# facebookresearch/esm

Measured on AMD Instinct MI355X. Metric: residues/sec (whole node) ESM-2 650M L=1022 bulk extract, higher is better.
Workload: dtype f16; 1 GPU; esm2_t33_650M_UR50D forward (repr_layers=[33] + logits), synthetic tokens [B,1024], random-init weights of the 650M architecture; batch_per_gpu=64, seq_len=1022, ln_fold=on (library default)

## Files before the change

### esm_amd/csrc/gemm9.hip

```cpp
#include "gemm_epi.h"
#include <type_traits>

namespace esmk {

constexpr int Q_BUF = 65536;
constexpr int Q_WOFF = 32768;
constexpr int Q_EPI = 2 * Q_BUF;
constexpr int Q_SLICE = 8192;
constexpr int Q_LDS = Q_EPI + 4 * Q_SLICE;

#define ESMK_INL __attribute__((always_inline))

template <typename T, int EPI, bool FULL, int D = 4, bool NT = true, int NMI = 8, bool SB = false, bool LNF = false>
ESMK_DEV void epilogue9_f32(const GemmArgs& p, f32x4 (&acc)[8][NMI], int m_base, int n_base, int lane, char* wl) {
    static_assert(!LNF || EPI == EPI_RESID_F32, "the LayerNorm-fold producer is the residual epilogue");
    constexpr bool lnp = LNF;
    constexpr int NP = 2 * NMI;
    constexpr int NIB = NMI / 2;
    float s1[4], s2[4];
    float cmv[2][4];
    typedef unsigned u32x2 __attribute__((ext_vector_type(2)));
    typedef unsigned u32x4 __attribute__((ext_vector_type(4)));
    u32x2 hold[4];
    T* h16 = reinterpret_cast<T*>(p.h16);
    if constexpr (!FULL)
        if (n_base >= p.N || m_base >= p.M) return;
    float* out = reinterpret_cast<float*>(p.out);
    const int ldc = p.N;
    const int g4 = lane >> 4, l16 = lane & 15;
    f32x4 old[D][4];
    constexpr bool SADDR = LNF && FULL;
    int la = lane;
    if constexpr (LNF) asm volatile("" : "+v"(la));
    typedef unsigned long long u64;
    u64 ob = 0, hb = 0, pb = 0, mb = 0;
    unsigned ov[4], hv[4];
    unsigned o_rb = 0, h_rb = 0, p_rb = 0;
    if constexpr (SADDR) {
        ob = (u64)out + ((u64)m_base * (u64)ldc + (u64)n_base) * 4;
        hb = (u64)h16 + ((u64)m_base * (u64)p.ldh + (u64)n_base) * sizeof(T);
        pb = (u64)p.ln_part + ((u64)m_base * (u64)p.ln_parts + (u64)(n_base >> 7)) * 8;
        mb = (u64)(p.ln_mean + m_base);
        o_rb = 32u * (unsigned)ldc, h_rb = 8u * (unsigned)sizeof(T) * (unsigned)p.ldh, p_rb = 64u * (unsigned)p.ln_parts;
        const unsigned r8 = la >> 3, c8 = la & 7;
#pragma unroll
        for (int it = 0; it < 4; ++it) {
            ov[it] = (8u * it + r8) * 4u * (unsigned)ldc + 16u * c8;
            hv[it] = (8u * it + r8) * (unsigned)sizeof(T) * (unsigned)p.ldh + (unsigned)sizeof(T) * ((c8 & 1) ? 32u + 4u * (c8 - 1) : 4u * c8);
        }
    }
    auto gaddr = [](u64 base, int imm, unsigned off, auto* as) ESMK_INL {
        asm("" : "+s"(base));
        typedef typename std::remove_pointer<decltype(as)>::type E;
        return (__attribute__((address_space(1))) E*)(base + (u64)imm + (u64)off);
    };
    auto out_at = [&](int i, int jb, int it) ESMK_INL { return gaddr(ob + (u64)(4 * i) * o_rb, 128 * jb, ov[it], (f32x4*)nullptr); };
    auto load_old = [&](f32x4 (&dst)[4], int piece) ESMK_INL {
        const int i = piece >> 2, jb = piece & 3;
        if constexpr (SADDR) {
#pragma unroll
            for (int it = 0; it < 4; ++it) dst[it] = *out_at(i, jb, it);
            return;
        }
#pragma unroll
        for (int it = 0; it < 4; ++it) {
            const int pc = it * 64 + la;
            const int m = FULL ? m_base + 32 * i + (pc >> 3) : min(m_base + 32 * i + (pc >> 3), p.M - 1);
            const int n = FULL ? n_base + 32 * jb + (pc & 7) * 4 : min(n_base + 32 * jb + (pc & 7) * 4, p.N - 4);
            dst[it] = *reinterpret_cast<const f32x4*>(out + (size_t)m * ldc + n);
        }
    };
    if constexpr (EPI == EPI_RESID_F32) {
#pragma unroll
        for (int d = 0; d < D; ++d) load_old(old[d], d);
    }
    auto load_means = [&](int i) ESMK_INL {
#pragma unroll
        for (int it = 0; it < 4; ++it) {
            const int m = m_base + 32 * i + it * 8 + (la >> 3);
            if constexpr (SADDR)
                cmv[i & 1][it] = (kExperiments && (p.lnf_dbg & 4)) ? 0.f : *gaddr(mb, 4 * (32 * i + 8 * it), 4u * (unsigned)(la >> 3), (const float*)nullptr);
            else
                cmv[i & 1][it] = (kExperiments && (p.lnf_dbg & 4)) ? 0.f : p.ln_mean[FULL ? m : min(m, p.M - 1)];
        }
    };
    if constexpr (LNF)
        if (lnp) load_means(0);
#pragma unroll
    for (int piece = 0; piece < NP; ++piece) {
        const int i = piece >> 2, jb = piece & 3;
        char* sl = wl + (SB ? 0 : (piece & 1) * 4096);
        if constexpr (LNF) {
            if (jb == 0 && lnp) {
#pragma unroll
                for (int it = 0; it < 4; ++it) s1[it] = s2[it] = 0.f;
                if (i + 1 < NIB) load_means(i + 1);
            }
        }
#pragma unroll
        for (int q = 0; q < 4; ++q) {
            const int mi2 = q >> 1, nj2 = q & 1;
            const int row = 16 * mi2 + l16;
            f32x4 v = acc[2 * jb + nj2][2 * i + mi2];
            if constexpr (EPI == EPI_GELU_F32) gelu_fast_x4(v);
            *reinterpret_cast<f32x4*>(sl + row * 128 + (((4 * nj2 + g4) ^ (row & 7)) << 4)) = v;
        }
        f32x4 vv[4];
#pragma unroll
        for (int it = 0; it < 4; ++it) {
            const int pc = it * 64 + lane;
            const int r = pc >> 3, cc = pc & 7;
            vv[it] = *reinterpret_cast<const f32x4*>(sl + r * 128 + ((cc ^ (r & 7)) << 4));
        }
#pragma unroll
        for (int it = 0; it < 4; ++it) {
            const int pc = it * 64 + la;
            const int r = pc >> 3, cc = pc & 7;
            f32x4 v = vv[it];
            if constexpr (EPI == EPI_RESID_F32) {
                const f32x4 o = old[piece % D][it];
                v = f32x4{o[0] + v[0], o[1] + v[1], o[2] + v[2], o[3] + v[3]};
            }
            const int m = m_base + 32 * i + r, n = n_base + 32 * jb + cc * 4;
            const bool inside = FULL || (m < p.M && n < p.N);
            if (inside) {
                if constexpr (SADDR) {
                    if constexpr (NT) __builtin_nontemporal_store(v, out_at(i, jb, it));
                    else *out_at(i, jb, it) = v;
                } else {
                    if constexpr (NT) __builtin_nontemporal_store(v, reinterpret_cast<f32x4*>(out + (size_t)m * ldc + n));
                    else *reinterpret_cast<f32x4*>(out + (size_t)m * ldc + n) = v;
                }
            }
            if (LNF && lnp) {
                const float c = cmv[i & 1][it];
                float d0 = v[0] - c, d1 = v[1] - c, d2 = v[2] - c, d3 = v[3] - c;
                if (!inside) d0 = d1 = d2 = d3 = 0.f;
                s1[it] += (d0 + d1) + (d2 + d3);
                s2[it] = __builtin_fmaf(d3, d3, __builtin_fmaf(d2, d2, __builtin_fmaf(d1, d1, __builtin_fmaf(d0, d0, s2[it]))));
                typename Op<T>::v4 pk;
                pk[0] = Op<T>::from(d0), pk[1] = Op<T>::from(d1), pk[2] = Op<T>::from(d2), pk[3] = Op<T>::from(d3);
                const u32x2 cur = __builtin_bit_cast(u32x2, pk);
                if ((jb & 1) == 0) {
                    hold[it] = cur;
                } else {
                    const bool odd = (lane & 1) != 0;
                    const u32x2 prev = hold[it];
                    const u32x2 send = odd ? prev : cur;
                    u32x2 recv;
                    recv.x = (unsigned)__builtin_amdgcn_update_dpp(0, (int)send.x, 0xB1, 0xf, 0xf, true);
                    recv.y = (unsigned)__builtin_amdgcn_update_dpp(0, (int)send.y, 0xB1, 0xf, 0xf, true);
                    const u32x4 o = odd ? u32x4{recv.x, recv.y, cur.x, cur.y} : u32x4{prev.x, prev.y, recv.x, recv.y};
                    const int col = n_base + ((la & 1) ? 32 * jb + 4 * (cc - 1) : 32 * (jb - 1) + 4 * cc);
                    if ((FULL || (m < p.M && col < p.N)) && !(kExperiments && (p.lnf_dbg & 1))) {
                        if constexpr (SADDR) {
                            auto* hd = gaddr(hb + (u64)(4 * i) * h_rb, 32 * (jb - 1) * (int)sizeof(T), hv[it], (u32x4*)nullptr);
                            if constexpr (NT) __builtin_nontemporal_store(o, hd);
                            else *hd = o;
                        } else {
                            auto* hd = reinterpret_cast<u32x4*>(h16 + (size_t)m * p.ldh + col);
                            if constexpr (NT) __builtin_nontemporal_store(o, hd);
                            else *hd = o;
                        }
                    }
                }
            }
        }
        if constexpr (EPI == EPI_RESID_F32)
            if (piece + D < NP) load_old(old[piece % D], piece + D);
        if constexpr (LNF) {
            if (jb == 3 && lnp && !(kExperiments && (p.lnf_dbg & 2))) {
#pragma unroll
                for (int it = 0; it < 4; ++it) {
                    float a = s1[it], b = s2[it];
                    a += __builtin_bit_cast(float, __builtin_amdgcn_update_dpp(0, __builtin_bit_cast(int, a), 0x111, 0xf, 0xf, true));
                    b += __builtin_bit_cast(float, __builtin_amdgcn_update_dpp(0, __builtin_bit_cast(int, b), 0x111, 0xf, 0xf, true));
                    a += __builtin_bit_cast(float, __builtin_amdgcn_update_dpp(0, __builtin_bit_cast(int, a), 0x112, 0xf, 0xf, true));
                    b += __builtin_bit_cast(float, __builtin_amdgcn_update_dpp(0, __builtin_bit_cast(int, b), 0x112, 0xf, 0xf, true));
                    a += __builtin_bit_cast(float, __builtin_amdgcn_update_dpp(0, __builtin_bit_cast(int, a), 0x114, 0xf, 0xf, true));
                    b += __builtin_bit_cast(float, __builtin_amdgcn_update_dpp(0, __builtin_bit_cast(int, b), 0x114, 0xf, 0xf, true));
                    const int m = m_base + 32 * i + it * 8 + (la >> 3);
                    if ((lane & 7) == 7 && (FULL || m < p.M)) {
                        f32x2 st = {a, b};
                        if constexpr (SADDR) {
                            *gaddr(pb + (u64)(4 * i + it) * p_rb, 0, (unsigned)(la >> 3) * 8u * (unsigned)p.ln_parts, (f32x2*)nullptr) = st;
                        } else {
                            *reinterpret_cast<f32x2*>(p.ln_part + ((size_t)m * p.ln_parts + (n_base >> 7)) * 2) = st;
                        }
                    }
                }
            }
        }
    }
}

template <typename T, int EPI, bool FULL, bool NT = false, int NMI = 8, int RR = 32, bool LNF = false, bool X3O = false>
ESMK_DEV void epilogue9_t(const GemmArgs& p, f32x4 (&acc)[8][NMI], int m_base, int n_base, int lane, char* wl) {
    static_assert(!X3O || (EPI == EPI_GELU_T && !LNF), "hi | hi | lo output rows: the plain GELU epilogue");
    using V8 = typename Op<T>::v8;
    float bs1[8];
    constexpr int LPR = EPI == EPI_QKV_ROPE ? 4 : 8;
    constexpr int RPI = 64 / LPR;
    constexpr int NIT = RR / RPI;
    constexpr int NI_ = NMI * 16 / RR;
    float rsv[LNF ? NI_ : 1][NIT];
    if constexpr (LNF) {
        if (FULL || m_base < p.M) {
#pragma unroll
            for (int i = 0; i < NI_; ++i)
#pragma unroll
                for (int it = 0; it < NIT; ++it) {
                    const int m = m_base + RR * i + RPI * it + lane / LPR;
                    rsv[i][it] = p.ln_rstd[FULL ? m : min(m, p.M - 1)];
                }
        }
    }
    constexpr int NI = NMI * 16 / RR;
    constexpr int NR = 2 * NI;
    constexpr int MB = RR / 16;
    const int g4 = lane >> 4, l16 = lane & 15;
    if constexpr (!FULL)
        if (m_base >= p.M) return;
    constexpr bool ROPE = EPI == EPI_QKV_ROPE;
    constexpr int NV = ROPE ? NI * NIT : 1;
    int rtt[NV];
    unsigned rro[NV];
    f32x4 tab[ROPE ? NIT : 1][4];
    float bsq1[ROPE && LNF ? 2 : 1][8], bsq2[ROPE && LNF ? 2 : 1][8];
    float sch[2] = {1.0f, 1.0f};
    T* qkh[2] = {nullptr, nullptr};
    int headh[2] = {0, 0};
    auto load_tab = [&](int it, int i) ESMK_INL {
        const size_t o = (size_t)rtt[i * NIT + it] * 32 + 8 * (lane & 3);
#pragma unroll
        for (int e2 = 0; e2 < 2; ++e2) {
            tab[it][e2] = *reinterpret_cast<const f32x4*>(p.cos + o + 4 * e2);
            tab[it][2 + e2] = *reinterpret_cast<const f32x4*>(p.sin + o + 4 * e2);
        }
    };
    if constexpr (ROPE) {
#pragma unroll
        for (int v = 0; v < NV; ++v) {
            const int mm = m_base + RR * (v / NIT) + 16 * (v % NIT) + (lane >> 2);
            const int m = FULL ? mm : min(mm, p.M - 1);
            const int b = m / p.T;
            rtt[v] = m - b * p.T;
            rro[v] = (unsigned)(b * p.H) * (unsigned)p.T + (unsigned)rtt[v];
        }
        if (p.row_pos != nullptr) {
#pragma unroll
            for (int v = 0; v < NV; ++v) {
                const int mm = m_base + RR * (v / NIT) + 16 * (v % NIT) + (lane >> 2);
                rtt[v] = p.row_pos[FULL ? mm : min(mm, p.M - 1)];
            }
        }
#pragma unroll
        for (int hf = 0; hf < 2; ++hf) {
            const int nb = n_base + 64 * hf;
            const bool live = FULL || nb < p.N;
            const int which = nb / p.E;
            headh[hf] = (nb - which * p.E) >> 6;
            qkh[hf] = reinterpret_cast<T*>(which == 0 ? p.q : p.k);
            sch[hf] = which == 0 ? p.scaling : 1.0f;
            if constexpr (LNF) {
                const int c0 = (live ? nb : n_base) + 8 * (lane & 3);
                f32x4 a[2], b[2];
#pragma unroll
                for (int e2 = 0; e2 < 2; ++e2)
                    a[e2] = *reinterpret_cast<const f32x4*>(p.bias + c0 + 4 * e2), b[e2] = *reinterpret_cast<const f32x4*>(p.bias + c0 + 32 + 4 * e2);
                if (p.bias2 != nullptr) {
#pragma unroll
                    for (int e2 = 0; e2 < 2; ++e2) {
                        const f32x4 a2 = *reinterpret_cast<const f32x4*>(p.bias2 + c0 + 4 * e2), b2 = *reinterpret_cast<const f32x4*>(p.bias2 + c0 + 32 + 4 * e2);
#pragma unroll
                        for (int e = 0; e < 4; ++e) a[e2][e] += a2[e], b[e2][e] += b2[e];
                    }
                }
#pragma unroll
                for (int e2 = 0; e2 < 2; ++e2)
#pragma unroll
                    for (int e = 0; e < 4; ++e) bsq1[hf][4 * e2 + e] = a[e2][e] * sch[hf], bsq2[hf][4 * e2 + e] = b[e2][e] * sch[hf];
            }
        }
#pragma unroll
        for (int it = 0; it < NIT; ++it) load_tab(it, 0);
    }
    auto write_round = [&](int r) ESMK_INL {
        const int hf = ROPE ? r % 2 : r / NI, i = ROPE ? r / 2 : r % NI;
#pragma unroll
        for (int mi2 = 0; mi2 < MB; ++mi2)
#pragma unroll
            for (int nq = 0; nq < 4; ++nq) {
                const int row = 16 * mi2 + l16, chunk = 4 * nq + g4;
                *reinterpret_cast<f32x4*>(wl + row * 256 + ((chunk ^ (row & 7)) << 4)) = acc[4 * hf + nq][MB * i + mi2];
            }
    };
    auto read_round = [&](f32x4 (&raw)[8]) ESMK_INL {
        if constexpr (EPI == EPI_QKV_ROPE) {
#pragma unroll
            for (int it = 0; it < RR / 16; ++it) {
                const int slot = it * 64 + lane;
                const int r = slot >> 2, g4 = slot & 3;
#pragma unroll
                for (int e2 = 0; e2 < 2; ++e2) {
                    raw[4 * it + e2] = *reinterpret_cast<const f32x4*>(wl + r * 256 + (((2 * g4 + e2) ^ (r & 7)) << 4));
                    raw[4 * it + 2 + e2] = *reinterpret_cast<const f32x4*>(wl + r * 256 + (((8 + 2 * g4 + e2) ^ (r & 7)) << 4));
                }
            }
        } else {
#pragma unroll
            for (int it = 0; it < RR / 8; ++it) {
                const int slot = it * 64 + lane;
                const int r = slot >> 3, c8 = slot & 7;
#pragma unroll
                for (int e2 = 0; e2 < 2; ++e2)
                    raw[2 * it + e2] = *reinterpret_cast<const f32x4*>(wl + r * 256 + (((2 * c8 + e2) ^ (r & 7)) << 4));
            }
        }
    };
    auto finish_round = [&](int rd, const f32x4 (&raw)[8]) ESMK_INL {
        const int hf = ROPE ? rd % 2 : rd / NI, i = ROPE ? rd / 2 : rd % NI;
        const int nb = n_base + 64 * hf;
        if constexpr (ROPE) {
            const bool live = FULL || nb < p.N;
            const float sc = sch[hf];
#pragma unroll
            for (int it = 0; it < NIT; ++it) {
                const int g4 = lane & 3;
                const int mm = m_base + RR * i + 16 * it + (lane >> 2);
                float rs = sc;
                if constexpr (LNF) rs = rsv[i][it] * sc;
                V8 o1, o2;
                if (live) {
                    float y1[8], y2[8];
#pragma unroll
                    for (int e2 = 0; e2 < 2; ++e2) {
                        const f32x4 c = tab[it][e2], s = tab[it][2 + e2];
#pragma unroll
                        for (int e = 0; e < 4; ++e) {
                            const float x1 = LNF ? __builtin_fmaf(raw[4 * it + e2][e], rs, bsq1[LNF ? hf : 0][4 * e2 + e]) : raw[4 * it + e2][e] * sc;
                            const float x2 = LNF ? __builtin_fmaf(raw[4 * it + 2 + e2][e], rs, bsq2[LNF ? hf : 0][4 * e2 + e]) : raw[4 * it + 2 + e2][e] * sc;
                            y1[4 * e2 + e] = __builtin_fmaf(x1, c[e], -(x2 * s[e]));
                            y2[4 * e2 + e] = __builtin_fmaf(x2, c[e], x1 * s[e]);
                        }
                    }
#pragma unroll
                    for (int e = 0; e < 8; ++e) o1[e] = Op<T>::from(y1[e]), o2[e] = Op<T>::from(y2[e]);
                }
                __builtin_amdgcn_sched_barrier(0);
                if (hf == 1 && i + 1 < NI) load_tab(it, i + 1);
                __builtin_amdgcn_sched_barrier(0);
                if (live && (FULL || mm < p.M)) {
                    T* dst = qkh[hf] + ((size_t)rro[i * NIT + it] + (size_t)headh[hf] * p.T) * 64 + 8 * g4;
                    if constexpr (NT) {
                        __builtin_nontemporal_store(o1, reinterpret_cast<V8*>(dst));
                        __builtin_nontemporal_store(o2, reinterpret_cast<V8*>(dst + 32));
                    } else {
                        *reinterpret_cast<V8*>(dst) = o1;
                        *reinterpret_cast<V8*>(dst + 32) = o2;
                    }
                }
            }
        } else {
            if constexpr (!FULL)
                if (nb >= p.N) return;
            T* out = reinterpret_cast<T*>(p.out);
            if constexpr (LNF) {
                if (i == 0) {
                    const int c0 = FULL ? nb + 8 * (lane & 7) : min(nb + 8 * (lane & 7), p.N - 8);
#pragma unroll
                    for (int e2 = 0; e2 < 2; ++e2) {
                        f32x4 a = *reinterpret_cast<const f32x4*>(p.bias + c0 + 4 * e2);
                        if (p.bias2 != nullptr) {
                            const f32x4 a2 = *reinterpret_cast<const f32x4*>(p.bias2 + c0 + 4 * e2);
#pragma unroll
                            for (int e = 0; e < 4; ++e) a[e] += a2[e];
                        }
#pragma unroll
                        for (int e = 0; e < 4; ++e) bs1[4 * e2 + e] = a[e];
                    }
                }
            }
#pragma unroll
            for (int it = 0; it < RR / 8; ++it) {
                const int slot = it * 64 + lane;
                const int r = slot >> 3, c8 = slot & 7;
                float v[8];
#pragma unroll
                for (int e2 = 0; e2 < 2; ++e2)
#pragma unroll
                    for (int e = 0; e < 4; ++e) v[4 * e2 + e] = raw[2 * it + e2][e];
                if constexpr (LNF) {
                    const float rs = rsv[i][it];
#pragma unroll
                    for (int e = 0; e < 8; ++e) v[e] = __builtin_fmaf(v[e], rs, bs1[e]);
                }
                if constexpr (EPI == EPI_GELU_T) gelu_fast_x8<!X3O>(v);
                V8 o;
#pragma unroll
                for (int e = 0; e < 8; ++e) o[e] = Op<T>::from(v[e]);
                const int m = m_base + RR * i + r, n = nb + 8 * c8;
                if constexpr (X3O) {
                    if (FULL || (m < p.M && n < p.N)) {
                        V8 lo;
#pragma unroll
                        for (int e = 0; e < 8; ++e) lo[e] = Op<T>::from(v[e] - Op<T>::to(o[e]));
                        T* q = out + (size_t)m * (3 * (size_t)p.N) + (size_t)(n >> 6) * 192 + (n & 63);
                        *reinterpret_cast<V8*>(q) = o;
                        *reinterpret_cast<V8*>(q + 64) = o;
                        *reinterpret_cast<V8*>(q + 128) = lo;
                    }
                } else
                if (FULL || (m < p.M && n < p.N)) {
                    if constexpr (NT) __builtin_nontemporal_store(o, reinterpret_cast<V8*>(out + (size_t)m * p.N + n));
                    else *reinterpret_cast<V8*>(out + (size_t)m * p.N + n) = o;
                }
            }
        }
    };
    write_round(0);
#pragma unroll
    for (int rd = 0; rd < NR; ++rd) {
        f32x4 raw[8];
        read_round(raw);
        if (rd + 1 < NR) write_round(rd + 1);
        __builtin_amdgcn_sched_barrier(0);
        finish_round(rd, raw);
    }
}

template <typename T, bool FULL, bool NT, int NMI, bool LNF, bool COL0>
ESMK_DEV void epilogue9_vt(const GemmArgs& p, f32x4 (&acc)[8][NMI], int m_base, int n_base, int lane, char* wl, int col0) {
    using V8 = typename Op<T>::v8;
    constexpr int NTH = NMI / 4;
    constexpr int CH = NMI == 8 ? 32 : 16;
    constexpr int NCG = 128 / CH;
    constexpr int NR = NTH * NCG;
    constexpr int NIT = CH / 8;
    const int g4 = lane >> 4, l16 = lane & 15;
    const int c8 = lane & 7, r8 = lane >> 3;
    const int ncols = COL0 ? p.N - col0 : p.N;
    if constexpr (!FULL)
        if (m_base >= p.M || n_base >= ncols) return;
    T* vt = reinterpret_cast<T*>(p.vt);
    const bool aligned = FULL || (p.T % 32 == 0);
    float bvc[NCG][NIT];
#pragma unroll
    for (int cg = 0; cg < NCG; ++cg)
#pragma unroll
        for (int it = 0; it < NIT; ++it) {
            const int n = n_base + CH * cg + 8 * it + r8;
            bvc[cg][it] = p.bias[(COL0 ? col0 : 0) + (FULL ? n : min(n, ncols - 1))];
        }
    if constexpr (LNF) {
        if (p.bias2 != nullptr) {
#pragma unroll
            for (int cg = 0; cg < NCG; ++cg)
#pragma unroll
                for (int it = 0; it < NIT; ++it) {
                    const int n = n_base + CH * cg + 8 * it + r8;
                    bvc[cg][it] += p.bias2[(COL0 ? col0 : 0) + (FULL ? n : min(n, ncols - 1))];
                }
        }
    }
    f32x4 rs[LNF ? NTH : 1][2];
    if constexpr (LNF) {
#pragma unroll
        for (int th = 0; th < NTH; ++th)
#pragma unroll
            for (int e2 = 0; e2 < 2; ++e2)
                rs[th][e2] = *reinterpret_cast<const f32x4*>(p.ln_rstd + m_base + 64 * th + 16 * (c8 >> 1) + 4 * ((c8 & 1) + 2 * e2));
    }
    size_t run[NTH];
#pragma unroll
    for (int th = 0; th < NTH; ++th) {
        const int m = m_base + 64 * th + 8 * c8;
        const int mc = FULL ? m : min(m, p.M - 1);
        const int b = mc / p.T;
        run[th] = (size_t)(b * p.H * 64) * p.Tp + (mc - b * p.T);
    }
    auto write_round = [&](int r) ESMK_INL {
        const int th = r / NCG, cg = r % NCG;
#pragma unroll
        for (int nj2 = 0; nj2 < CH / 16; ++nj2)
#pragma unroll
            for (int mq = 0; mq < 4; ++mq) {
                const int row = 16 * nj2 + l16, chunk = 4 * mq + g4;
                *reinterpret_cast<f32x4*>(wl + row * 256 + ((chunk ^ (row & 7)) << 4)) = acc[(CH / 16) * cg + nj2][4 * th + mq];
            }
    };
    auto read_round = [&](f32x4 (&raw)[2 * NIT]) ESMK_INL {
#pragma unroll
        for (int it = 0; it < NIT; ++it) {
            const int r = 8 * it + r8;
#pragma unroll
            for (int e2 = 0; e2 < 2; ++e2)
                raw[2 * it + e2] = *reinterpret_cast<const f32x4*>(wl + r * 256 + (((4 * (c8 >> 1) + (c8 & 1) + 2 * e2) ^ (r & 7)) << 4));
        }
    };
    size_t eo[8];
    auto finish_round = [&](int rd, const f32x4 (&raw)[2 * NIT]) ESMK_INL {
        const int th = rd / NCG, cg = rd % NCG;
        if constexpr (!FULL) {
            if (n_base + CH * cg >= ncols) return;
            if (!aligned && cg == 0) {
#pragma unroll
                for (int e2 = 0; e2 < 2; ++e2)
#pragma unroll
                    for (int e = 0; e < 4; ++e) {
                        const int m = m_base + 64 * th + 16 * (c8 >> 1) + 4 * ((c8 & 1) + 2 * e2) + e;
                        const int mc = min(m, p.M - 1);
                        const int b = mc / p.T, t = mc - b * p.T;
                        const int t16 = t & 15;
                        const int tp = (t & ~15) | ((((t16 >> 2) & 1) << 3) | (((t16 >> 3) & 1) << 2) | (t16 & 3));
                        eo[4 * e2 + e] = m < p.M ? (size_t)(b * p.H * 64) * p.Tp + tp : ~(size_t)0;
                    }
            }
        }
#pragma unroll
        for (int it = 0; it < NIT; ++it) {
            const int n = n_base + CH * cg + 8 * it + r8;
            const float bv = bvc[cg][it];
            float x[8];
#pragma unroll
            for (int e2 = 0; e2 < 2; ++e2)
#pragma unroll
                for (int e = 0; e < 4; ++e) {
                    if constexpr (LNF) x[4 * e2 + e] = __builtin_fmaf(raw[2 * it + e2][e], rs[th][e2][e], bv);
                    else x[4 * e2 + e] = raw[2 * it + e2][e] + bv;
                }
            asm volatile("" : "+v"(x[0]), "+v"(x[1]), "+v"(x[2]), "+v"(x[3]), "+v"(x[4]), "+v"(x[5]), "+v"(x[6]), "+v"(x[7]));
            V8 o;
#pragma unroll
            for (int e = 0; e < 8; ++e) o[e] = Op<T>::from(x[e]);
            if (aligned) {
                if (FULL || (m_base + 64 * th + 8 * c8 < p.M && n < ncols)) {
                    T* dst = vt + run[th] + (size_t)n * p.Tp;
                    if constexpr (NT) __builtin_nontemporal_store(o, reinterpret_cast<V8*>(dst));
                    else *reinterpret_cast<V8*>(dst) = o;
                }
            } else if constexpr (!FULL) {
                if (n < ncols) {
#pragma unroll
                    for (int e = 0; e < 8; ++e)
                        if (eo[e] != ~(size_t)0) vt[eo[e] + (size_t)n * p.Tp] = o[e];
                }
            }
        }
    };
    write_round(0);
#pragma unroll
    for (int rd = 0; rd < NR; ++rd) {
        f32x4 raw[2 * NIT];
        read_round(raw);
        if (rd + 1 < NR) write_round(rd + 1);
        __builtin_amdgcn_sched_barrier(0);
        finish_round(rd, raw);
    }
}

template <typename T, int EPI, int VAR = 0, bool HM = false, bool LNF = false, bool X3O = false>
__global__ __launch_bounds__(256, 1) void gemm9_kernel(GemmArgs p, unsigned long long* timing) {
    static_assert(!X3O || (EPI == EPI_GELU_T && !HM && !LNF && VAR == 0), "hi | hi | lo output rows: plain full-height GELU kernel");
    static_assert(!LNF || EPI == EPI_RESID_F32 || EPI == EPI_QKV_ROPE || EPI == EPI_V_T || EPI == EPI_GELU_T || EPI == EPI_QKV_ALL,
                  "LayerNorm fold: epilogue");
    constexpr bool LNC = LNF && EPI != EPI_RESID_F32;
    using VtDefault = std::integral_constant<bool, EPI == EPI_V_T>;
    constexpr int TM = HM ? 128 : 256;
    constexpr int NMI = HM ? 4 : 8;
    constexpr int NPC = NMI + 8;
    constexpr int NRD = NMI + 8;
    constexpr int NS = 8 * NMI;
    constexpr int NST = HM ? 3 : 2;
    constexpr int BUF = HM ? 49152 : Q_BUF, WOFF = HM ? 16384 : Q_WOFF;
    constexpr int SLICE = HM ? 4096 : Q_SLICE;
    static_assert(NST * BUF + 4 * SLICE <= Q_LDS, "LDS budget");
    static_assert(!HM || (VAR & ~(8 | 16 | 32 | 64 | 128)) == 0, "half-height tiles: only the timing-experiment bits");
    extern __shared__ __attribute__((aligned(16))) char smem[];
    using V8 = typename Op<T>::v8;
    typedef __attribute__((address_space(3))) void* lds_ptr;
    constexpr bool NO_MFMA = (VAR & 16) != 0, NO_DMA = (VAR & 32) != 0, NO_RD = (VAR & 64) != 0, NO_EPI = (VAR & 128) != 0;
    constexpr int IMODE = VAR & 3;
    constexpr int M_B1 = HM ? 8 : (IMODE == 0 ? 16 : 24);
    constexpr int M_B2 = HM ? 16 : 52;
    constexpr bool STAGGER = (VAR & 4) != 0;
    constexpr bool NO_BAR = (VAR & 8) != 0;
#ifndef ESMK_G9_TIE1
#define ESMK_G9_TIE1 1
#endif
    constexpr bool TIE1 = ESMK_G9_TIE1 && !HM && !NO_MFMA;
    constexpr int KSTAG = (VAR & 256) ? 1 : (VAR & 512) ? 2 : 0;
    constexpr bool HALF_DMA = (VAR & 1024) != 0;
    constexpr int DMA_AUX = (VAR & 2048) ? 2 : 0;
    auto piece_slot = [](int k) constexpr {
        if (HM) return 8 + 2 * k;
        return IMODE == 3 ? 24 + 2 * k : IMODE == 1 ? 24 + k : IMODE == 2 ? 24 + (k * 40) / 16 : 16 + 3 * k;
    };
    auto pieces_before = [piece_slot](int m) constexpr {
        int n = 0;
        for (int k = 0; k < NPC; ++k) n += piece_slot(k) < m ? 1 : 0;
        return n;
    };
    constexpr int IN_FLIGHT0 = pieces_before(M_B2);
    constexpr int IN_FLIGHT = HALF_DMA ? (IN_FLIGHT0 + 1) / 2 : IN_FLIGHT0 + (HM ? NPC : 0);
    const int tid = threadIdx.x;
    const int lane = tid & 63;
    const int wave = __builtin_amdgcn_readfirstlane(tid >> 6);
    const int wr = wave >> 1, wc = wave & 1;
    const int nk = p.K >> 6;
    const unsigned rb = (unsigned)p.K * 2u;
    const unsigned rb_a = p.a_row_bytes ? (unsigned)p.a_row_bytes : rb;
    const bool a_rep = p.a_kt_repeat != 0;

    const int tiles_m = (p.M + TM - 1) / TM, tiles_n = (p.N + 255) >> 8;
    const int total = tiles_m * tiles_n;
    const int xcd = blockIdx.x & 7, slot = blockIdx.x >> 3, nslot = gridDim.x >> 3;
    const int q8 = total >> 3, r8 = total & 7;
    const int start = (xcd < r8) ? xcd * (q8 + 1) : r8 * (q8 + 1) + (xcd - r8) * q8;
    const int cnt = q8 + (xcd < r8 ? 1 : 0);
    const int n_my = (cnt > slot) ? (cnt - slot + nslot - 1) / nslot : 0;
    if (n_my == 0) return;
    const int panel_c = p.panel_c > 0 ? p.panel_c : tiles_n;
    const int panel_full = tiles_m * panel_c;
    auto tile_coords = [&](int it, int& tmi, int& tni) ESMK_INL {
        const int o = start + slot + it * nslot;
        const int pnl = o / panel_full;
        const int rem = o - pnl * panel_full;
        const int w = min(panel_c, tiles_n - pnl * panel_c);
        tmi = __builtin_amdgcn_readfirstlane(rem / w);
        tni = __builtin_amdgcn_readfirstlane(pnl * panel_c + (rem - tmi * w));
    };

    auto uniform_ptr = [](const void* ptr) ESMK_INL {
        const unsigned long long a = (unsigned long long)ptr;
        const unsigned lo = __builtin_amdgcn_readfirstlane((unsigned)a), hi = __builtin_amdgcn_readfirstlane((unsigned)(a >> 32));
        return (void*)(((unsigned long long)hi << 32) | lo);
    };
    __amdgpu_buffer_rsrc_t d_a, d_w;
    int s_kt, s_it;
    unsigned s_koff, s_koff_a;
    const unsigned rb8 = 8u * rb, rb8_a = 8u * rb_a;
    const unsigned vo_base = (unsigned)(64 * wave + (lane >> 3)) * rb;
    const unsigned vo_even = vo_base + (unsigned)(((lane & 7) ^ ((lane >> 4) & 3)) << 4);
    const unsigned vo_odd = vo_base + (unsigned)(((lane & 7) ^ (4 + ((lane >> 4) & 3))) << 4);
    const unsigned va_base = (unsigned)((HM ? 32 : 64) * wave + (lane >> 3)) * rb_a;
    const unsigned va_even = va_base + (unsigned)(((lane & 7) ^ ((lane >> 4) & 3)) << 4);
    const unsigned va_odd = va_base + (unsigned)(((lane & 7) ^ (4 + ((lane >> 4) & 3))) << 4);
    auto set_tile = [&](int it) ESMK_INL {
        int tmi, tni;
        tile_coords(it, tmi, tni);
        s_it = it;
        s_kt = 0;
        if constexpr (KSTAG == 1) s_koff = (unsigned)(((blockIdx.x >> 3) & 3) * (nk >> 2)) * 128u;
        else if constexpr (KSTAG == 2) s_koff = (unsigned)((tni & 3) * (nk >> 2)) * 128u;
        else s_koff = 0;
        s_koff_a = a_rep ? 0u : s_koff;
        const unsigned rows_a = (unsigned)min(TM, p.M - tmi * TM), rows_w = (unsigned)min(256, p.N - tni * 256);
        d_a = __builtin_amdgcn_make_buffer_rsrc(uniform_ptr(reinterpret_cast<const char*>(p.A) + (size_t)tmi * TM * rb_a), 0,
                                                (int)__builtin_amdgcn_readfirstlane(rows_a * rb_a), 0x00020000);
        d_w = __builtin_amdgcn_make_buffer_rsrc(uniform_ptr(reinterpret_cast<const char*>(p.W) + (size_t)tni * 256 * rb), 0,
                                                (int)__builtin_amdgcn_readfirstlane(rows_w * rb), 0x00020000);
    };
    auto advance = [&]() ESMK_INL {
        if (s_kt + 1 < nk) {
            s_kt = s_kt + 1;
            s_koff += 128u;
            if constexpr (KSTAG != 0)
                if (s_koff == (unsigned)nk * 128u) s_koff = 0;
            s_koff_a = a_rep ? (unsigned)(s_kt >> 1) * 128u : s_koff;
        } else if (s_it + 1 < n_my) {
            set_tile(s_it + 1);
        }
    };
    auto issue1 = [&](int k, int buf) ESMK_INL {
        if constexpr (!NO_DMA) {
            if constexpr (HALF_DMA)
                if (k & 1) return;
            const bool isw = HM ? (k >= 4) : ((k & 1) != 0);
            const int q = HM ? (isw ? k - 4 : k) : (k >> 1);
            char* dst = smem + buf * BUF + (isw ? WOFF + wave * 8192 : wave * (HM ? 4096 : 8192)) + q * 1024;
            __builtin_amdgcn_raw_ptr_buffer_load_lds(isw ? d_w : d_a, (lds_ptr)dst, 16,
                                                     isw ? ((q & 1) ? vo_odd : vo_even) : ((q & 1) ? va_odd : va_even),
                                                     isw ? s_koff + (unsigned)q * rb8 : s_koff_a + (unsigned)q * rb8_a, 0, DMA_AUX);
        }
    };

    const int lrow = (lane & 15) * 128;
    const int swz = (lane >> 1) & 7;
    int xo[2];
#pragma unroll
    for (int hf = 0; hf < 2; ++hf) xo[hf] = ((4 * hf + (lane >> 4)) ^ swz) << 4;
    const int a_off = wr * (NMI * 2048) + lrow;
    const int w_off = WOFF + wc * 16384 + lrow;
    V8 xa[NMI], xw[8], ya[NMI], yw[8];
    if constexpr (NO_RD) {
#pragma unroll
        for (int i = 0; i < 8; ++i)
#pragma unroll
            for (int e = 0; e < 8; ++e) {
                xw[i][e] = yw[i][e] = Op<T>::from(0.f);
                if (i < NMI) xa[i][e] = ya[i][e] = Op<T>::from(0.f);
            }
    }
    auto rd1 = [&](V8 (&fa)[NMI], V8 (&fw)[8], const char* bp, int half, int r) ESMK_INL {
        if constexpr (!NO_RD) {
            if (r >= 2 * NMI) {
                const int blk = r - NMI;
                fw[blk] = *reinterpret_cast<const V8*>(bp + w_off + blk * 2048 + xo[half]);
            } else {
                const int blk = r >> 1;
                if (r & 1) fw[blk] = *reinterpret_cast<const V8*>(bp + w_off + blk * 2048 + xo[half]);
                else fa[blk] = *reinterpret_cast<const V8*>(bp + a_off + blk * 2048 + xo[half]);
            }
        }
    };

    f32x4 acc[8][NMI];
    f32x4 bv[8];
    auto load_bias = [&](int n_base) ESMK_INL {
        bool done = false;
        if constexpr (EPI != EPI_V_T && !LNC) {
            bool want = p.bias != nullptr;
            if constexpr (EPI == EPI_QKV_ALL) want = want && n_base < 2 * p.E;
            if (want) {
                int lb = lane;
                if constexpr (LNF && EPI == EPI_RESID_F32) asm volatile("" : "+v"(lb));
                const int g4 = lb >> 4;
                if (n_base + 128 <= p.N) {
#pragma unroll
                    for (int nj = 0; nj < 8; ++nj) bv[nj] = *reinterpret_cast<const f32x4*>(p.bias + n_base + 16 * nj + 4 * g4);
                } else {
#pragma unroll
                    for (int nj = 0; nj < 8; ++nj)
#pragma unroll
                        for (int r = 0; r < 4; ++r) {
                            const int n = n_base + 16 * nj + 4 * g4 + r;
                            bv[nj][r] = n < p.N ? p.bias[n] : 0.f;
                        }
                }
                done = true;
            }
        }
        if (!done) {
#pragma unroll
            for (int nj = 0; nj < 8; ++nj) bv[nj] = f32x4{0.f, 0.f, 0.f, 0.f};
        }
    };
    auto mma1 = [&](const V8 (&fa)[NMI], const V8 (&fw)[8], int m, auto first_t, auto vt, auto half_t) ESMK_INL {
        constexpr bool first = decltype(first_t)::value;
        constexpr bool second_half = decltype(half_t)::value;
#pragma unroll
        for (int pp = 0; pp < 2; ++pp) {
            const int idx = 2 * (m % (NS / 2)) + pp;
            const int nj = idx / NMI, mi = idx % NMI;
            f32x4& c = acc[nj][mi];
            const bool use_b = first && m < NS / 2;
            constexpr bool tied = TIE1 && first && second_half;
            if constexpr (NO_MFMA) {
                asm volatile("" ::"v"(fa[mi]), "v"(fw[nj]));
                if (use_b) c = bv[nj];
            } else if constexpr (TIE1 && first) {
                if constexpr (tied) {
                    if constexpr (decltype(vt)::value) Op<T>::mma16_tied(fa[mi], fw[nj], c);
                    else Op<T>::mma16_tied(fw[nj], fa[mi], c);
                } else if constexpr (decltype(vt)::value) {
                    c = Op<T>::mma16(fa[mi], fw[nj], bv[nj]);
                } else {
                    c = Op<T>::mma16(fw[nj], fa[mi], bv[nj]);
                }
            } else if constexpr (decltype(vt)::value) {
                c = use_b ? Op<T>::mma16(fa[mi], fw[nj], bv[nj]) : Op<T>::mma16(fa[mi], fw[nj], c);
            } else {
                c = use_b ? Op<T>::mma16(fw[nj], fa[mi], bv[nj]) : Op<T>::mma16(fw[nj], fa[mi], c);
            }
        }
    };

    int cur = 0;
    auto ktile = [&](auto first, auto vt) ESMK_INL {
        const int nxt = (cur + 1 == NST) ? 0 : cur + 1;
        const char* sb = smem + cur * BUF;
        const char* sn = smem + nxt * BUF;
        advance();
        __builtin_amdgcn_sched_barrier(0);
#pragma unroll
        for (int m = 0; m < NS; ++m) {
            if (m == M_B1) {
                if constexpr (NO_BAR) asm volatile("s_waitcnt lgkmcnt(0)" ::: "memory");
                else asm volatile("s_waitcnt lgkmcnt(0)\n\ts_barrier" ::: "memory");
                __builtin_amdgcn_sched_barrier(0);
            }
            if (m == M_B2) {
                if constexpr (NO_BAR) asm volatile("s_waitcnt vmcnt(%0)" ::"n"(IN_FLIGHT) : "memory");
                else asm volatile("s_waitcnt vmcnt(%0)\n\ts_barrier" ::"n"(IN_FLIGHT) : "memory");
                __builtin_amdgcn_sched_barrier(0);
            }
            if (m < NS / 2) mma1(xa, xw, m, first, vt, std::false_type{});
            else mma1(ya, yw, m, first, vt, std::true_type{});
            if constexpr (HM) {
                if (m < NRD / 2) {
                    rd1(ya, yw, sb, 1, 2 * m);
                    rd1(ya, yw, sb, 1, 2 * m + 1);
                }
            } else {
                if (m < NRD) rd1(ya, yw, sb, 1, m);
            }
            if constexpr (STAGGER) {
                if (m >= M_B1 && m < M_B1 + 32 && ((m - M_B1) & 1) == 0) {
                    if (!(wave & 1)) issue1((m - M_B1) >> 1, cur);
                } else if (m > M_B1 && m < M_B1 + 33 && ((m - M_B1) & 1) == 1) {
                    if (wave & 1) issue1((m - M_B1 - 1) >> 1, cur);
                }
            } else {
#pragma unroll
                for (int k = 0; k < NPC; ++k)
                    if (piece_slot(k) == m) issue1(k, cur);
            }
            if constexpr (M_B2 + NRD <= NS) {
                if (m >= M_B2 && m < M_B2 + NRD) rd1(xa, xw, sn, 0, m - M_B2);
            } else {
                if (m >= M_B2 && m < M_B2 + NRD / 2) {
                    rd1(xa, xw, sn, 0, 2 * (m - M_B2));
                    rd1(xa, xw, sn, 0, 2 * (m - M_B2) + 1);
                }
            }
            __builtin_amdgcn_sched_barrier(0);
        }
        if constexpr (LNF && EPI == EPI_RESID_F32 && !HM) {
#pragma unroll
            for (int nj = 0; nj < 8; ++nj)
#pragma unroll
                for (int mi = 0; mi < NMI; ++mi) asm volatile("" : "+a"(acc[nj][mi]));
        }
        if constexpr (TIE1 && decltype(first)::value) asm volatile("s_nop 7\n\ts_nop 7");
        cur = nxt;
    };

    set_tile(0);
#pragma unroll
    for (int k = 0; k < NPC; ++k) issue1(k, 0);
#pragma unroll
    for (int st = 1; st < NST; ++st) {
        advance();
#pragma unroll
        for (int k = 0; k < NPC; ++k) issue1(k, st);
    }
    if constexpr (EPI == EPI_RESID_F32 && !HM && VAR == 0) {
        if (p.desync > 0) {
            const int g = p.desync_group == 0 ? (int)(blockIdx.x & 1) : p.desync_group == 1 ? (int)((blockIdx.x >> 3) & 1) : (int)(blockIdx.x & 3);
            const long long wait = p.desync_group == 2 ? (long long)g * p.desync / 2 : (long long)g * p.desync;
            if (wait > 0) {
                const unsigned long long t0 = __builtin_readcyclecounter();
                while ((long long)(__builtin_readcyclecounter() - t0) < wait) __builtin_amdgcn_s_sleep(32);
            }
        }
    }
    asm volatile("s_waitcnt vmcnt(%0)\n\ts_barrier" ::"n"(HALF_DMA ? 8 : (NST - 1) * NPC) : "memory");
    __builtin_amdgcn_sched_barrier(0);
#pragma unroll
    for (int r = 0; r < NRD; ++r) rd1(xa, xw, smem, 0, r);

    auto stamp = [&](int it, int k) ESMK_INL {
        if (timing != nullptr && tid == 0) {
            unsigned long long* t = timing + ((size_t)blockIdx.x * 32 + (it & 31)) * 4;
            t[k] = __builtin_readcyclecounter();
            if (k == 2) t[3] = wall_clock64();
        }
    };

    {
        int tmi, tni;
        tile_coords(0, tmi, tni);
        load_bias(tni * 256 + wc * 128);
    }
    for (int it = 0; it < n_my; ++it) {
        int tmi, tni;
        tile_coords(it, tmi, tni);
        constexpr int WRM = TM / 2;
        const int m_base = tmi * TM + wr * WRM, n_base = tni * 256 + wc * 128;
        stamp(it, 0);
        bool v_tile = false;
        if constexpr (EPI == EPI_QKV_ALL) v_tile = tni * 256 >= 2 * p.E;
        if constexpr (EPI == EPI_QKV_ALL) {
            if (v_tile) {
                ktile(std::true_type{}, std::true_type{});
#pragma unroll 1
                for (int kt = 1; kt < nk; ++kt) ktile(std::false_type{}, std::true_type{});
            } else {
                ktile(std::true_type{}, std::false_type{});
#pragma unroll 1
                for (int kt = 1; kt < nk; ++kt) ktile(std::false_type{}, std::false_type{});
            }
        } else {
            ktile(std::true_type{}, VtDefault{});
#pragma unroll 1
            for (int kt = 1; kt < nk; ++kt) ktile(std::false_type{}, VtDefault{});
        }
        stamp(it, 1);
        constexpr bool BIAS_EARLY = (EPI == EPI_STORE_T || EPI == EPI_GELU_T);
        auto next_bias = [&]() ESMK_INL {
            if (it + 1 < n_my) {
                int tm2, tn2;
                tile_coords(it + 1, tm2, tn2);
                load_bias(tn2 * 256 + wc * 128);
            } else if constexpr (LNF && EPI == EPI_RESID_F32) {
#pragma unroll
                for (int nj = 0; nj < 8; ++nj) bv[nj] = f32x4{0.f, 0.f, 0.f, 0.f};
            }
        };
        if constexpr (BIAS_EARLY) next_bias();
        char* slice = smem + NST * BUF + wave * SLICE;
        const bool full = (m_base + WRM <= p.M) && (n_base + 128 <= p.N);
        constexpr bool NTS = !HM && (VAR & 4096) == 0;
        if constexpr (NO_EPI) {
#pragma unroll
            for (int nj = 0; nj < 8; ++nj)
#pragma unroll
                for (int mi = 0; mi < NMI; ++mi) asm volatile("" ::"a"(acc[nj][mi]));
        } else if constexpr (EPI == EPI_STORE_F32 || EPI == EPI_GELU_F32 || EPI == EPI_RESID_F32) {
            constexpr int RD = LNF ? 3 : 4;
            if (full) epilogue9_f32<T, EPI, true, RD, NTS, NMI, HM, LNF>(p, acc, m_base, n_base, lane, slice);
            else epilogue9_f32<T, EPI, false, RD, NTS, NMI, HM, LNF>(p, acc, m_base, n_base, lane, slice);
        } else if constexpr (EPI == EPI_V_T) {
            if (full && p.T % 32 == 0) epilogue9_vt<T, true, NTS, NMI, LNF, false>(p, acc, m_base, n_base, lane, slice, 0);
            else epilogue9_vt<T, false, NTS, NMI, LNF, false>(p, acc, m_base, n_base, lane, slice, 0);
        } else if constexpr (EPI == EPI_QKV_ALL) {
            if (v_tile) {
                const int col0 = 2 * p.E;
                if (full && p.T % 32 == 0) epilogue9_vt<T, true, NTS, NMI, LNF, true>(p, acc, m_base, n_base - col0, lane, slice, col0);
                else epilogue9_vt<T, false, NTS, NMI, LNF, true>(p, acc, m_base, n_base - col0, lane, slice, col0);
            } else {
                if (full) epilogue9_t<T, EPI_QKV_ROPE, true, NTS, NMI, HM ? 16 : 32, LNF>(p, acc, m_base, n_base, lane, slice);
                else epilogue9_t<T, EPI_QKV_ROPE, false, NTS, NMI, HM ? 16 : 32, LNF>(p, acc, m_base, n_base, lane, slice);
            }
        } else {
            if (full) epilogue9_t<T, EPI, true, NTS, NMI, HM ? 16 : 32, LNF, X3O>(p, acc, m_base, n_base, lane, slice);
            else epilogue9_t<T, EPI, false, NTS, NMI, HM ? 16 : 32, LNF, X3O>(p, acc, m_base, n_base, lane, slice);
        }
        if constexpr (!BIAS_EARLY) next_bias();
        stamp(it, 2);
    }
    wait_vmcnt0();
}

static unsigned long long* g_timing9 = nullptr;
void gemm9_set_timing(unsigned long long* dev_buf) { g_timing9 = dev_buf; }

static int num_workgroups9() {
    static int n = 0;
    if (n == 0) {
        int dev = 0, cus = 0;
        if (hipGetDevice(&dev) != hipSuccess ||
            hipDeviceGetAttribute(&cus, hipDeviceAttributeMultiprocessorCount, dev) != hipSuccess || cus < 8)
            cus = 256;
        n = cus / 8 * 8;
    }
    return n;
}

template <typename T, int EPI, int VAR = 0, bool HM = false, bool LNF = false, bool X3O = false>
static hipError_t launch9(GemmArgs p, hipStream_t st) {
    static bool attr_set = false;
    auto kern = gemm9_kernel<T, EPI, VAR, HM, LNF, X3O>;
    if (!attr_set) {
        hipError_t e = hipFuncSetAttribute(reinterpret_cast<const void*>(kern),
                                           hipFuncAttributeMaxDynamicSharedMemorySize, Q_LDS);
        if (e != hipSuccess) return e;
        attr_set = true;
    }
    const int tiles_n = (p.N + 255) / 256;
    if (p.panel_c <= 0) {
        if (tiles_n <= 6) p.panel_c = tiles_n;
        else if (tiles_n % 5 == 0) p.panel_c = 5;
        else if (tiles_n % 4 == 0) p.panel_c = 4;
        else if (tiles_n % 6 == 0) p.panel_c = 6;
        else p.panel_c = 5;
    }
    hipLaunchKernelGGL(kern, dim3(num_workgroups9()), dim3(256), Q_LDS, st, p, g_timing9);
    return hipGetLastError();
}

bool gemm9_ln_fold(const GemmArgs& p, int epi) {
    if (epi == EPI_RESID_F32) return p.ln_part != nullptr;
    if (epi == EPI_QKV_ROPE || epi == EPI_V_T || epi == EPI_GELU_T || epi == EPI_QKV_ALL) return p.ln_rstd != nullptr;
    return false;
}

bool gemm9_supports(const GemmArgs& p, int epi) {
    if (p.K % 64 != 0 || p.N % 8 != 0 || p.M <= 0) return false;
    if (p.w_row_bytes || p.a_kt_bytes || p.w_kt_bytes || p.batch > 1 || p.n_valid > 0 || p.ldc > 0 || p.row_keep != nullptr ||
        p.vt_rows > 0 || p.rowmap_R > 0 || epi == EPI_MSA_CTX || p.head_dim != 64)
        return false;
    if (gemm9_ln_fold(p, epi) && p.a_kt_repeat) return false;
    if (p.x3_out && (epi != EPI_GELU_T || p.N % 64 != 0)) return false;
    if (p.a_row_bytes && (p.a_row_bytes % 16 != 0)) return false;
    if ((epi == EPI_QKV_ROPE || epi == EPI_V_T) && p.N % 64 != 0) return false;
    if (epi == EPI_QKV_ALL && !(p.E > 0 && p.E % 128 == 0 && p.N == 3 * p.E && !p.a_kt_repeat && !p.a_row_bytes && p.bias != nullptr))
        return false;
    if ((long long)256 * p.K * 2 > 0x7fffffffLL) return false;
    return (epi >= EPI_STORE_T && epi <= EPI_V_T) || epi == EPI_QKV_ALL;
}

template <typename T>
static hipError_t dispatch9(const GemmArgs& p, int epi, int var, hipStream_t st) {
#ifdef ESMK_EXPERIMENTS
#define ESMK_G9_ALL(V)                                                       \
    switch (epi) {                                                            \
        case EPI_STORE_T: return launch9<T, EPI_STORE_T, V>(p, st);           \
        case EPI_STORE_F32: return launch9<T, EPI_STORE_F32, V>(p, st);       \
        case EPI_GELU_T: return launch9<T, EPI_GELU_T, V>(p, st);             \
        case EPI_GELU_F32: return launch9<T, EPI_GELU_F32, V>(p, st);         \
        case EPI_RESID_F32: return launch9<T, EPI_RESID_F32, V>(p, st);       \
        case EPI_QKV_ROPE: return launch9<T, EPI_QKV_ROPE, V>(p, st);         \
        case EPI_V_T: return launch9<T, EPI_V_T, V>(p, st);                   \
    }
    if (var == 2) { ESMK_G9_ALL(2) }
    if (var == 3) { ESMK_G9_ALL(3) }
#undef ESMK_G9_ALL
    if constexpr (std::is_same<T, _Float16>::value) {
        if (p.half_m > 0 && epi == EPI_STORE_T) {
            switch (var) {
                case 8: return launch9<T, EPI_STORE_T, 8, true>(p, st);
                case 16: return launch9<T, EPI_STORE_T, 16, true>(p, st);
                case 32: return launch9<T, EPI_STORE_T, 32, true>(p, st);
                case 64: return launch9<T, EPI_STORE_T, 64, true>(p, st);
                case 128: return launch9<T, EPI_STORE_T, 128, true>(p, st);
                case 96: return launch9<T, EPI_STORE_T, 96, true>(p, st);
                case 224: return launch9<T, EPI_STORE_T, 224, true>(p, st);
            }
        }
    }
#else
    if (var != 0) return hipErrorInvalidValue;
#endif
    if (p.x3_out) {
        if constexpr (std::is_same<T, _Float16>::value) {
            if (epi == EPI_GELU_T && var == 0 && !gemm9_ln_fold(p, epi)) return launch9<T, EPI_GELU_T, 0, false, false, true>(p, st);
        }
        return hipErrorInvalidValue;
    }
    if (gemm9_ln_fold(p, epi)) {
        if (var != 0) return hipErrorInvalidValue;
        if (epi == EPI_RESID_F32 && (p.h16 == nullptr || p.ln_mean == nullptr || p.ldh < p.N || p.ln_parts < (p.N + 127) / 128))
            return hipErrorInvalidValue;
        if (epi != EPI_RESID_F32 && p.bias == nullptr) return hipErrorInvalidValue;
        if (p.half_m > 0) {
            switch (epi) {
                case EPI_RESID_F32: return launch9<T, EPI_RESID_F32, 0, true, true>(p, st);
                case EPI_QKV_ROPE: return launch9<T, EPI_QKV_ROPE, 0, true, true>(p, st);
                case EPI_V_T: return launch9<T, EPI_V_T, 0, true, true>(p, st);
                case EPI_GELU_T: return launch9<T, EPI_GELU_T, 0, true, true>(p, st);
                case EPI_QKV_ALL: return launch9<T, EPI_QKV_ALL, 0, true, true>(p, st);
            }
        }
        switch (epi) {
            case EPI_RESID_F32: return launch9<T, EPI_RESID_F32, 0, false, true>(p, st);
            case EPI_QKV_ROPE: return launch9<T, EPI_QKV_ROPE, 0, false, true>(p, st);
            case EPI_V_T: return launch9<T, EPI_V_T, 0, false, true>(p, st);
            case EPI_GELU_T: return launch9<T, EPI_GELU_T, 0, false, true>(p, st);
            case EPI_QKV_ALL: return hipErrorInvalidValue;
        }
        return hipErrorInvalidValue;
    }
    if (var == 0 && p.half_m > 0) {
        switch (epi) {
            case EPI_STORE_T: return launch9<T, EPI_STORE_T, 0, true>(p, st);
            case EPI_STORE_F32: return launch9<T, EPI_STORE_F32, 0, true>(p, st);
            case EPI_GELU_T: return launch9<T, EPI_GELU_T, 0, true>(p, st);
            case EPI_GELU_F32: return launch9<T, EPI_GELU_F32, 0, true>(p, st);
            case EPI_RESID_F32: return launch9<T, EPI_RESID_F32, 0, true>(p, st);
            case EPI_QKV_ROPE: return launch9<T, EPI_QKV_ROPE, 0, true>(p, st);
            case EPI_V_T: return launch9<T, EPI_V_T, 0, true>(p, st);
            case EPI_QKV_ALL: return launch9<T, EPI_QKV_ALL, 0, true>(p, st);
        }
    }
    if (var == 0) {
        switch (epi) {
            case EPI_STORE_T: return launch9<T, EPI_STORE_T>(p, st);
            case EPI_STORE_F32: return launch9<T, EPI_STORE_F32>(p, st);
            case EPI_GELU_T: return launch9<T, EPI_GELU_T>(p, st);
            case EPI_GELU_F32: return launch9<T, EPI_GELU_F32>(p, st);
            case EPI_RESID_F32: return launch9<T, EPI_RESID_F32>(p, st);
            case EPI_QKV_ROPE: return launch9<T, EPI_QKV_ROPE>(p, st);
            case EPI_V_T: return launch9<T, EPI_V_T>(p, st);
            case EPI_QKV_ALL: return hipErrorInvalidValue;
        }
    }
#ifdef ESMK_EXPERIMENTS
    if constexpr (std::is_same<T, _Float16>::value) {
        if (epi == EPI_STORE_T) {
            switch (var) {
                case 1: return launch9<T, EPI_STORE_T, 1>(p, st);
                case 7: return launch9<T, EPI_STORE_T, 7>(p, st);
                case 512: return launch9<T, EPI_STORE_T, 512>(p, st);
                case 2048: return launch9<T, EPI_STORE_T, 2048>(p, st);
                case 4096: return launch9<T, EPI_STORE_T, 4096>(p, st);
                case 8: return launch9<T, EPI_STORE_T, 8>(p, st);
                case 16: return launch9<T, EPI_STORE_T, 16>(p, st);
                case 32: return launch9<T, EPI_STORE_T, 32>(p, st);
                case 64: return launch9<T, EPI_STORE_T, 64>(p, st);
                case 128: return launch9<T, EPI_STORE_T, 128>(p, st);
                case 96: return launch9<T, EPI_STORE_T, 96>(p, st);
                case 224: return launch9<T, EPI_STORE_T, 224>(p, st);
                case 1040: return launch9<T, EPI_STORE_T, 1040>(p, st);
            }
        }
    }
#endif
    return hipErrorInvalidValue;
}

hipError_t launch_gemm9(const GemmArgs& p, int epi, int operand_dtype, int var, hipStream_t st) {
    if (!gemm9_supports(p, epi)) return hipErrorInvalidValue;
    if (operand_dtype == ESMK_DT_F16) return dispatch9<_Float16>(p, epi, var, st);
    if (operand_dtype == ESMK_DT_BF16) return dispatch9<__bf16>(p, epi, var, st);
    return hipErrorInvalidValue;
}

}
```

Baseline: 720,000 residues/s.

## Double-buffer LDS epilogue rounds for LayerNorm-folded GELU GEMM

For the LayerNorm-folded GELU epilogue in the full-height kernel, the round size drops to 16 rows. Two 4 KiB LDS images are kept in flight, so the read of the next round and the write of the round after overlap the arithmetic and stores of the current one. The folded bias is preloaded once for both halves instead of per round. Debug flags that skip stores, LDS traffic or arithmetic are also added, gated behind kExperiments. The change costs more registers for the doubled raw buffers and bias, which may hurt scheduling or occupancy.

New measurement: 721,600 residues/s (median of 6 runs). Within noise of the previous version (+0.2%).

```diff
diff --git a/esm_amd/csrc/gemm9.hip b/esm_amd/csrc/gemm9.hip
--- a/esm_amd/csrc/gemm9.hip
+++ b/esm_amd/csrc/gemm9.hip
@@ -194,11 +194,30 @@
     }
 }
 
-template <typename T, int EPI, bool FULL, bool NT = false, int NMI = 8, int RR = 32, bool LNF = false, bool X3O = false>
+template <typename T, int EPI, bool FULL, bool NT = false, int NMI = 8, int RR = 32, bool LNF = false, bool X3O = false, bool TWO = false>
 ESMK_DEV void epilogue9_t(const GemmArgs& p, f32x4 (&acc)[8][NMI], int m_base, int n_base, int lane, char* wl) {
     static_assert(!X3O || (EPI == EPI_GELU_T && !LNF), "hi | hi | lo output rows: the plain GELU epilogue");
+    static_assert(!TWO || (RR == 16 && NMI == 8 && LNF && EPI == EPI_GELU_T), "two rounds in flight: two 4 KiB images in the 8 KiB slice");
     using V8 = typename Op<T>::v8;
-    float bs1[8];
+    constexpr bool BS2 = TWO;
+    float bs1[BS2 ? 2 : 1][8];
+    if constexpr (BS2) {
+        if (FULL || m_base < p.M) {
+            const float* b2p = p.bias2 != nullptr ? p.bias2 : p.bias;
+#pragma unroll
+            for (int hf = 0; hf < 2; ++hf) {
+                const int c0 = FULL ? n_base + 64 * hf + 8 * (lane & 7) : max(0, min(n_base + 64 * hf + 8 * (lane & 7), p.N - 8));
+#pragma unroll
+                for (int e2 = 0; e2 < 2; ++e2) {
+                    const f32x4 a = *reinterpret_cast<const f32x4*>(p.bias + c0 + 4 * e2);
+                    const f32x4 a2 = *reinterpret_cast<const f32x4*>(b2p + c0 + 4 * e2);
+#pragma unroll
+                    for (int e = 0; e < 4; ++e) bs1[hf][4 * e2 + e] = p.bias2 != nullptr ? a[e] + a2[e] : a[e];
+                }
+            }
+        }
+    }
+    const bool x_nost = kExperiments && (p.lnf_dbg & 8), x_nolds = kExperiments && (p.lnf_dbg & 16), x_noar = kExperiments && (p.lnf_dbg & 32);
     constexpr int LPR = EPI == EPI_QKV_ROPE ? 4 : 8;
     constexpr int RPI = 64 / LPR;
     constexpr int NIT = RR / RPI;
@@ -219,6 +238,7 @@
     constexpr int NR = 2 * NI;
     constexpr int MB = RR / 16;
     const int g4 = lane >> 4, l16 = lane & 15;
+    const char* const wl0 = wl;
     if constexpr (!FULL)
         if (m_base >= p.M) return;
     constexpr bool ROPE = EPI == EPI_QKV_ROPE;
@@ -285,17 +305,19 @@
 #pragma unroll
         for (int it = 0; it < NIT; ++it) load_tab(it, 0);
     }
-    auto write_round = [&](int r) ESMK_INL {
+    auto write_round = [&](int r, int img) ESMK_INL {
         const int hf = ROPE ? r % 2 : r / NI, i = ROPE ? r / 2 : r % NI;
+        char* wi = wl + img * (RR * 256);
 #pragma unroll
         for (int mi2 = 0; mi2 < MB; ++mi2)
 #pragma unroll
             for (int nq = 0; nq < 4; ++nq) {
                 const int row = 16 * mi2 + l16, chunk = 4 * nq + g4;
-                *reinterpret_cast<f32x4*>(wl + row * 256 + ((chunk ^ (row & 7)) << 4)) = acc[4 * hf + nq][MB * i + mi2];
-            }
-    };
-    auto read_round = [&](f32x4 (&raw)[8]) ESMK_INL {
+                *reinterpret_cast<f32x4*>(wi + row * 256 + ((chunk ^ (row & 7)) << 4)) = acc[4 * hf + nq][MB * i + mi2];
+            }
+    };
+    auto read_round = [&](f32x4 (&raw)[8], int img) ESMK_INL {
+        const char* wl = wl0 + img * (RR * 256);
         if constexpr (EPI == EPI_QKV_ROPE) {
 #pragma unroll
             for (int it = 0; it < RR / 16; ++it) {
@@ -331,7 +353,12 @@
                 float rs = sc;
                 if constexpr (LNF) rs = rsv[i][it] * sc;
                 V8 o1, o2;
-                if (live) {
+                if (live && x_noar) {
+#pragma unroll
+                    for (int e2 = 0; e2 < 2; ++e2)
+#pragma unroll
+                        for (int e = 0; e < 4; ++e) o1[4 * e2 + e] = Op<T>::from(raw[4 * it + e2][e]), o2[4 * e2 + e] = Op<T>::from(raw[4 * it + 2 + e2][e]);
+                } else if (live) {
                     float y1[8], y2[8];
 #pragma unroll
                     for (int e2 = 0; e2 < 2; ++e2) {
@@ -350,7 +377,9 @@
                 __builtin_amdgcn_sched_barrier(0);
                 if (hf == 1 && i + 1 < NI) load_tab(it, i + 1);
                 __builtin_amdgcn_sched_barrier(0);
-                if (live && (FULL || mm < p.M)) {
+                if (x_nost) {
+                    asm volatile("" ::"v"(o1), "v"(o2));
+                } else if (live && (FULL || mm < p.M)) {
                     T* dst = qkh[hf] + ((size_t)rro[i * NIT + it] + (size_t)headh[hf] * p.T) * 64 + 8 * g4;
                     if constexpr (NT) {
                         __builtin_nontemporal_store(o1, reinterpret_cast<V8*>(dst));
@@ -365,7 +394,7 @@
             if constexpr (!FULL)
                 if (nb >= p.N) return;
             T* out = reinterpret_cast<T*>(p.out);
-            if constexpr (LNF) {
+            if constexpr (LNF && !BS2) {
                 if (i == 0) {
                     const int c0 = FULL ? nb + 8 * (lane & 7) : min(nb + 8 * (lane & 7), p.N - 8);
 #pragma unroll
@@ -377,7 +406,7 @@
                             for (int e = 0; e < 4; ++e) a[e] += a2[e];
                         }
 #pragma unroll
-                        for (int e = 0; e < 4; ++e) bs1[4 * e2 + e] = a[e];
+                        for (int e = 0; e < 4; ++e) bs1[0][4 * e2 + e] = a[e];
                     }
                 }
             }
@@ -392,10 +421,12 @@
                     for (int e = 0; e < 4; ++e) v[4 * e2 + e] = raw[2 * it + e2][e];
                 if constexpr (LNF) {
                     const float rs = rsv[i][it];
-#pragma unroll
-                    for (int e = 0; e < 8; ++e) v[e] = __builtin_fmaf(v[e], rs, bs1[e]);
-                }
-                if constexpr (EPI == EPI_GELU_T) gelu_fast_x8<!X3O>(v);
+                    if (!x_noar)
+#pragma unroll
+                        for (int e = 0; e < 8; ++e) v[e] = __builtin_fmaf(v[e], rs, bs1[BS2 ? hf : 0][e]);
+                }
+                if constexpr (EPI == EPI_GELU_T)
+                    if (!x_noar) gelu_fast_x8<!X3O>(v);
                 V8 o;
 #pragma unroll
                 for (int e = 0; e < 8; ++e) o[e] = Op<T>::from(v[e]);
@@ -410,6 +441,8 @@
                         *reinterpret_cast<V8*>(q + 64) = o;
                         *reinterpret_cast<V8*>(q + 128) = lo;
                     }
+                } else if (x_nost) {
+                    asm volatile("" ::"v"(o));
                 } else
                 if (FULL || (m < p.M && n < p.N)) {
                     if constexpr (NT) __builtin_nontemporal_store(o, reinterpret_cast<V8*>(out + (size_t)m * p.N + n));
@@ -418,14 +451,38 @@
             }
         }
     };
-    write_round(0);
-#pragma unroll
-    for (int rd = 0; rd < NR; ++rd) {
-        f32x4 raw[8];
-        read_round(raw);
-        if (rd + 1 < NR) write_round(rd + 1);
-        __builtin_amdgcn_sched_barrier(0);
-        finish_round(rd, raw);
+    if (x_nolds) {
+#pragma unroll
+        for (int rd = 0; rd < NR; ++rd) {
+            f32x4 raw[8];
+#pragma unroll
+            for (int k = 0; k < 8; ++k) asm volatile("" : "=v"(raw[k]));
+            finish_round(rd, raw);
+        }
+        return;
+    }
+    if constexpr (TWO) {
+        f32x4 raw[2][8];
+        write_round(0, 0);
+        write_round(1, 1);
+        read_round(raw[0], 0);
+#pragma unroll
+        for (int rd = 0; rd < NR; ++rd) {
+            if (rd + 1 < NR) read_round(raw[(rd + 1) & 1], (rd + 1) & 1);
+            if (rd + 2 < NR) write_round(rd + 2, rd & 1);
+            __builtin_amdgcn_sched_barrier(0);
+            finish_round(rd, raw[rd & 1]);
+        }
+    } else {
+        write_round(0, 0);
+#pragma unroll
+        for (int rd = 0; rd < NR; ++rd) {
+            f32x4 raw[8];
+            read_round(raw, 0);
+            if (rd + 1 < NR) write_round(rd + 1, 0);
+            __builtin_amdgcn_sched_barrier(0);
+            finish_round(rd, raw);
+        }
     }
 }
 
@@ -498,6 +555,7 @@
                 raw[2 * it + e2] = *reinterpret_cast<const f32x4*>(wl + r * 256 + (((4 * (c8 >> 1) + (c8 & 1) + 2 * e2) ^ (r & 7)) << 4));
         }
     };
+    const bool x_nost = kExperiments && (p.lnf_dbg & 8), x_nolds = kExperiments && (p.lnf_dbg & 16), x_noar = kExperiments && (p.lnf_dbg & 32);
     size_t eo[8];
     auto finish_round = [&](int rd, const f32x4 (&raw)[2 * NIT]) ESMK_INL {
         const int th = rd / NCG, cg = rd % NCG;
@@ -526,14 +584,17 @@
             for (int e2 = 0; e2 < 2; ++e2)
 #pragma unroll
                 for (int e = 0; e < 4; ++e) {
-                    if constexpr (LNF) x[4 * e2 + e] = __builtin_fmaf(raw[2 * it + e2][e], rs[th][e2][e], bv);
+                    if (x_noar) x[4 * e2 + e] = raw[2 * it + e2][e];
+                    else if constexpr (LNF) x[4 * e2 + e] = __builtin_fmaf(raw[2 * it + e2][e], rs[th][e2][e], bv);
                     else x[4 * e2 + e] = raw[2 * it + e2][e] + bv;
                 }
             asm volatile("" : "+v"(x[0]), "+v"(x[1]), "+v"(x[2]), "+v"(x[3]), "+v"(x[4]), "+v"(x[5]), "+v"(x[6]), "+v"(x[7]));
             V8 o;
 #pragma unroll
             for (int e = 0; e < 8; ++e) o[e] = Op<T>::from(x[e]);
-            if (aligned) {
+            if (x_nost) {
+                asm volatile("" ::"v"(o));
+            } else if (aligned) {
                 if (FULL || (m_base + 64 * th + 8 * c8 < p.M && n < ncols)) {
                     T* dst = vt + run[th] + (size_t)n * p.Tp;
                     if constexpr (NT) __builtin_nontemporal_store(o, reinterpret_cast<V8*>(dst));
@@ -548,6 +609,16 @@
             }
         }
     };
+    if (x_nolds) {
+#pragma unroll
+        for (int rd = 0; rd < NR; ++rd) {
+            f32x4 raw[2 * NIT];
+#pragma unroll
+            for (int k = 0; k < 2 * NIT; ++k) asm volatile("" : "=v"(raw[k]));
+            finish_round(rd, raw);
+        }
+        return;
+    }
     write_round(0);
 #pragma unroll
     for (int rd = 0; rd < NR; ++rd) {
@@ -934,8 +1005,10 @@
                 else epilogue9_t<T, EPI_QKV_ROPE, false, NTS, NMI, HM ? 16 : 32, LNF>(p, acc, m_base, n_base, lane, slice);
             }
         } else {
-            if (full) epilogue9_t<T, EPI, true, NTS, NMI, HM ? 16 : 32, LNF, X3O>(p, acc, m_base, n_base, lane, slice);
-            else epilogue9_t<T, EPI, false, NTS, NMI, HM ? 16 : 32, LNF, X3O>(p, acc, m_base, n_base, lane, slice);
+            constexpr bool TWO = !HM && LNF && EPI == EPI_GELU_T;
+            constexpr int RR = (HM || TWO) ? 16 : 32;
+            if (full) epilogue9_t<T, EPI, true, NTS, NMI, RR, LNF, X3O, TWO>(p, acc, m_base, n_base, lane, slice);
+            else epilogue9_t<T, EPI, false, NTS, NMI, RR, LNF, X3O, TWO>(p, acc, m_base, n_base, lane, slice);
         }
         if constexpr (!BIAS_EARLY) next_bias();
         stamp(it, 2);
```
